# owensgroup/sparsify.me

Measured on AMD Instinct MI355X. Metric: effective GF/s (2:4 spmma vs dense gemm) on ResNet-50 layer shapes, higher is better.
Workload: dtype f16

## Files before the change

### sparsify.me_amd/csrc/mma_tile.h

```cpp
#pragma once
#include "sm_common.h"
#include "select24.h"

namespace sm {

typedef __attribute__((address_space(3))) char lds_char;
typedef __attribute__((address_space(3))) s4 lds_s4;

__device__ __forceinline__ unsigned a_off(unsigned row, unsigned chunk) {
  return row * 128u + 16u * (chunk ^ (row & 7u));
}

__device__ __forceinline__ unsigned b_swz(unsigned kr) { return (((kr >> 1) & 1u) << 1) | (((kr >> 3) & 1u) << 2); }
template <int KROWS>
__device__ __forceinline__ unsigned b_off(unsigned kr, unsigned col ) {
  const unsigned panel = col >> 6, cl = col & 63u;
  return panel * (KROWS * 128u) + kr * 128u + 16u * ((cl >> 3) ^ b_swz(kr)) + 2u * (cl & 7u);
}

template <int KROWS>
__device__ __forceinline__ s4 b_read_tr(const char* Bs, unsigned kr0, unsigned col0, unsigned lane) {
  const unsigned i = lane & 15u, q = i >> 2, p = i & 3u;
  const char* addr = Bs + b_off<KROWS>(kr0 + q, col0 + 4u * p);
  return __builtin_amdgcn_ds_read_tr16_b64_v4i16((lds_s4*)(lds_char*)addr);
// ... 15 lines not shown
}
template <bool BF>
__device__ __forceinline__ f4 smfmac16(h8 a, h16 b, f4 c, int idx) {
  if constexpr (BF) return __builtin_amdgcn_smfmac_f32_16x16x64_bf16(__builtin_bit_cast(bf8, a), __builtin_bit_cast(bf16x16, b), c, idx, 0, 0);
  else return __builtin_amdgcn_smfmac_f32_16x16x64_f16(a, b, c, idx, 0, 0);
}
template <bool BF>
__device__ __forceinline__ f4 mfma16(h8 a, h8 b, f4 c) {
  if constexpr (BF) return __builtin_amdgcn_mfma_f32_16x16x32_bf16(__builtin_bit_cast(bf8, a), __builtin_bit_cast(bf8, b), c, 0, 0, 0);
  else return __builtin_amdgcn_mfma_f32_16x16x32_f16(a, b, c, 0, 0, 0);
}

template <int FM, int FN, bool BF = false>
__device__ __forceinline__ void smfmac_stage(const char* As, const char* Ms, const char* Bs, unsigned row0, unsigned col0,
                                             unsigned lane, f4 (&acc)[FM][FN]) {
  const unsigned g = lane >> 4, r = lane & 15u;
  h8 af[FM];
  int idx[FM];
#pragma unroll
  for (int i = 0; i < FM; ++i) {
    const unsigned row = row0 + i * 16 + r;
    af[i] = *reinterpret_cast<const h8*>(As + row * 64u + 16u * (g ^ a64_swz(row)));
    idx[i] = (int)*reinterpret_cast<const unsigned short*>(Ms + row * 8u + 2u * g);
  }
  const unsigned bs_addr = (unsigned)(uintptr_t)(lds_char*)Bs;
  s4 t0[2], t1[2], t2[2], t3[2];
  auto issue = [&](int j, s4& v0, s4& v1, s4& v2, s4& v3) {
    const unsigned c0 = col0 + j * 16, q = r >> 2, pp = r & 3u;
    const unsigned a = bs_addr + b_off<64>(8u * g + q, c0 + 4u * pp);
    asm volatile("ds_read_b64_tr_b16 %0, %4\n\tds_read_b64_tr_b16 %1, %4 offset:512\n\t"
                 "ds_read_b64_tr_b16 %2, %4 offset:4096\n\tds_read_b64_tr_b16 %3, %4 offset:4608"
                 : "=&v"(v0), "=&v"(v1), "=&v"(v2), "=&v"(v3) : "v"(a) : "memory");
  };
  issue(0, t0[0], t1[0], t2[0], t3[0]);
#pragma unroll
  for (int j = 0; j < FN; ++j) {
    const int c = j & 1, n = c ^ 1;
    if (j + 1 < FN) {
      issue(j + 1, t0[n], t1[n], t2[n], t3[n]);
      asm volatile("s_waitcnt lgkmcnt(4)" : "+v"(t0[c]), "+v"(t1[c]), "+v"(t2[c]), "+v"(t3[c]) :: "memory");
    } else {
      asm volatile("s_waitcnt lgkmcnt(0)" : "+v"(t0[c]), "+v"(t1[c]), "+v"(t2[c]), "+v"(t3[c]) :: "memory");
    }
    __builtin_amdgcn_sched_barrier(0);
    typedef short s16 __attribute__((ext_vector_type(16)));
    const s16 all = {t0[c][0], t0[c][1], t0[c][2], t0[c][3], t1[c][0], t1[c][1], t1[c][2], t1[c][3],
                     t2[c][0], t2[c][1], t2[c][2], t2[c][3], t3[c][0], t3[c][1], t3[c][2], t3[c][3]};
    const h16 bf = __builtin_bit_cast(h16, all);
#pragma unroll
    for (int i = 0; i < FM; ++i) acc[i][j] = smfmac16<BF>(af[i], bf, acc[i][j], idx[i]);
  }
}

template <int FM, int FN, bool BF = false, int D = 1>
__device__ __forceinline__ void smfmac_b_sweep(const h8 (&af)[FM], const int (&idx)[FM], const char* Bs, unsigned col0, unsigned lane,
                                               f4 (&acc)[FM][FN]) {
  static_assert(D == 1 || D == 2, "fragments in flight");
  const unsigned g = lane >> 4, r = lane & 15u;
  const unsigned bs_addr = (unsigned)(uintptr_t)(lds_char*)Bs;
  s4 t0[D + 1], t1[D + 1], t2[D + 1], t3[D + 1];
  auto issue = [&](int j, s4& v0, s4& v1, s4& v2, s4& v3) {
    const unsigned c0 = col0 + j * 16, q = r >> 2, pp = r & 3u;
    const unsigned a = bs_addr + b_off<64>(8u * g + q, c0 + 4u * pp);
    asm volatile("ds_read_b64_tr_b16 %0, %4\n\tds_read_b64_tr_b16 %1, %4 offset:512\n\t"
                 "ds_read_b64_tr_b16 %2, %4 offset:4096\n\tds_read_b64_tr_b16 %3, %4 offset:4608"
                 : "=&v"(v0), "=&v"(v1), "=&v"(v2), "=&v"(v3) : "v"(a) : "memory");
  };
#pragma unroll
  for (int j = 0; j < D; ++j)
    if (j < FN) issue(j, t0[j], t1[j], t2[j], t3[j]);
#pragma unroll
  for (int j = 0; j < FN; ++j) {
    const int c = j % (D + 1), n = (j + D) % (D + 1);
    if (j + D < FN) {
      issue(j + D, t0[n], t1[n], t2[n], t3[n]);
      asm volatile("s_waitcnt lgkmcnt(%4)" : "+v"(t0[c]), "+v"(t1[c]), "+v"(t2[c]), "+v"(t3[c]) : "n"(4 * D) : "memory");
    } else if (D == 2 && j + 1 < FN) {
      asm volatile("s_waitcnt lgkmcnt(4)" : "+v"(t0[c]), "+v"(t1[c]), "+v"(t2[c]), "+v"(t3[c]) :: "memory");
    } else {
      asm volatile("s_waitcnt lgkmcnt(0)" : "+v"(t0[c]), "+v"(t1[c]), "+v"(t2[c]), "+v"(t3[c]) :: "memory");
    }
    __builtin_amdgcn_sched_barrier(0);
    typedef short s16 __attribute__((ext_vector_type(16)));
    const s16 all = {t0[c][0], t0[c][1], t0[c][2], t0[c][3], t1[c][0], t1[c][1], t1[c][2], t1[c][3],
                     t2[c][0], t2[c][1], t2[c][2], t2[c][3], t3[c][0], t3[c][1], t3[c][2], t3[c][3]};
    const h16 bf = __builtin_bit_cast(h16, all);
#pragma unroll
    for (int i = 0; i < FM; ++i) acc[i][j] = smfmac16<BF>(af[i], bf, acc[i][j], idx[i]);
  }
}

__device__ __forceinline__ void dense16_to_operand(const u4 lo, const u4 hi, h8& af, int& idx) {
  uint32_t k0, k1, k2, k3, n0, n1, n2, n3;
  strip_select_f16(lo[0], lo[1], k0, n0);
  strip_select_f16(lo[2], lo[3], k1, n1);
  strip_select_f16(hi[0], hi[1], k2, n2);
  strip_select_f16(hi[2], hi[3], k3, n3);
  af = __builtin_bit_cast(h8, u4{k0, k1, k2, k3});
  idx = (int)(n0 | (n1 << 4) | (n2 << 8) | (n3 << 12));
}

template <int FM, int FN, bool BF = false, int D = 1>
__device__ __forceinline__ void smfmac_stage_dense_a(const char* Araw, const char* Bs, unsigned row0, unsigned col0,
                                                     unsigned lane, f4 (&acc)[FM][FN]) {
  const unsigned g = lane >> 4, r = lane & 15u;
  h8 af[FM];
  int idx[FM];
#pragma unroll
  for (int i = 0; i < FM; ++i) {
    const unsigned row = row0 + i * 16 + r;
    const u4 lo = *reinterpret_cast<const u4*>(Araw + a_off(row, 2u * g));
    const u4 hi = *reinterpret_cast<const u4*>(Araw + a_off(row, 2u * g + 1u));
    dense16_to_operand(lo, hi, af[i], idx[i]);
  }
  smfmac_b_sweep<FM, FN, BF, D>(af, idx, Bs, col0, lane, acc);
}

template <int FM, int FN, bool BF = false>
__device__ __forceinline__ void mfma_b_sweep(const h8 (&a0)[FM], const h8 (&a1)[FM], const char* Bs, unsigned col0, unsigned lane, f4 (&acc)[FM][FN]) {
  const unsigned g = lane >> 4, r = lane & 15u;
  const unsigned bs_addr = (unsigned)(uintptr_t)(lds_char*)Bs;
  s4 t0[2], t1[2], t2[2], t3[2];
  auto issue = [&](int j, s4& v0, s4& v1, s4& v2, s4& v3) {
    const unsigned c0 = col0 + j * 16, q = r >> 2, pp = r & 3u;
    const unsigned a = bs_addr + b_off<64>(8u * g + q, c0 + 4u * pp);
    asm volatile("ds_read_b64_tr_b16 %0, %4\n\tds_read_b64_tr_b16 %1, %4 offset:512\n\t"
                 "ds_read_b64_tr_b16 %2, %4 offset:4096\n\tds_read_b64_tr_b16 %3, %4 offset:4608"
                 : "=&v"(v0), "=&v"(v1), "=&v"(v2), "=&v"(v3) : "v"(a) : "memory");
  };
  issue(0, t0[0], t1[0], t2[0], t3[0]);
#pragma unroll
  for (int j = 0; j < FN; ++j) {
    const int c = j & 1, n = c ^ 1;
    if (j + 1 < FN) {
      issue(j + 1, t0[n], t1[n], t2[n], t3[n]);
      asm volatile("s_waitcnt lgkmcnt(4)" : "+v"(t0[c]), "+v"(t1[c]), "+v"(t2[c]), "+v"(t3[c]) :: "memory");
    } else {
      asm volatile("s_waitcnt lgkmcnt(0)" : "+v"(t0[c]), "+v"(t1[c]), "+v"(t2[c]), "+v"(t3[c]) :: "memory");
    }
    __builtin_amdgcn_sched_barrier(0);
    typedef short s8v __attribute__((ext_vector_type(8)));
    const s8v lo = {t0[c][0], t0[c][1], t0[c][2], t0[c][3], t1[c][0], t1[c][1], t1[c][2], t1[c][3]};
    const s8v hi = {t2[c][0], t2[c][1], t2[c][2], t2[c][3], t3[c][0], t3[c][1], t3[c][2], t3[c][3]};
    const h8 b0 = __builtin_bit_cast(h8, lo), b1 = __builtin_bit_cast(h8, hi);
#pragma unroll
    for (int i = 0; i < FM; ++i) acc[i][j] = mfma16<BF>(a0[i], b0, acc[i][j]);
#pragma unroll
    for (int i = 0; i < FM; ++i) acc[i][j] = mfma16<BF>(a1[i], b1, acc[i][j]);
  }
}
template <int FM, int FN, bool BF = false>
__device__ __forceinline__ void mfma_stage_dense_a(const char* Araw, const char* Bs, unsigned row0, unsigned col0, unsigned lane, f4 (&acc)[FM][FN]) {
  const unsigned g = lane >> 4, r = lane & 15u;
  h8 a0[FM], a1[FM];
#pragma unroll
  for (int i = 0; i < FM; ++i) {
    const unsigned row = row0 + i * 16 + r;
    a0[i] = *reinterpret_cast<const h8*>(Araw + a_off(row, g));
    a1[i] = *reinterpret_cast<const h8*>(Araw + a_off(row, 4u + g));
  }
  mfma_b_sweep<FM, FN, BF>(a0, a1, Bs, col0, lane, acc);
}

template <int BM, int BN, int FM, int FN, int NT, bool BF = false>
__device__ __forceinline__ void store_c_tile(char* smem, half_t* C, const f4 (&acc)[FM][FN], bool has_acc, unsigned row0,
                                             unsigned col0, int m0, int n0, int Mrows, int N, float alpha, float beta,
                                             unsigned tid) {
  constexpr int CPITCH = BN * 2 + 16;
// ... 67 lines not shown
      break;
    case SM_ACT_HARDSWISH:
#pragma unroll
      for (int q = 0; q < 4; ++q) {
        float t = x[q] + 3.0f;
        t = t > 0.0f ? (t < 6.0f ? t : 6.0f) : (t == t ? 0.0f : t);
        y[q] = (x[q] * t) * (1.0f / 6.0f);
      }
      break;
    default: break;
  }
  return y;
}

__device__ __forceinline__ f4 epi_bias4(f4 v, bool bias_col, float bj, bool bias_row, f4 bi) {
#pragma clang fp contract(off)
  if (bias_col) v += bj;
  if (bias_row) v += bi;
  return v;
}

template <int FM, int FN>
struct EpiBias {
  static constexpr int NV = FN > 4 * FM ? FN : 4 * FM;
  float v[NV];
};
template <int FM, int FN>
__device__ __forceinline__ EpiBias<FM, FN> epi_bias_prefetch(const EpiArgs& e, bool has_acc, unsigned row0, unsigned col0, int m0, int n0, int Mrows,
                                                            int N, unsigned lane) {
  EpiBias<FM, FN> eb;
  const unsigned g = lane >> 4, r = lane & 15u;
#pragma unroll
  for (int t = 0; t < EpiBias<FM, FN>::NV; ++t) eb.v[t] = 0.0f;
  if (has_acc && e.bias != nullptr) {
    if (e.bias_dim == SM_BIAS_COL) {
#pragma unroll
      for (int j = 0; j < FN; ++j) {
        const int gc = n0 + (int)(col0 + j * 16 + r);
        if (gc < N) eb.v[j] = e.bias[gc];
      }
    } else {
#pragma unroll
      for (int i = 0; i < FM; ++i)
#pragma unroll
        for (int q = 0; q < 4; ++q) {
          const int gr = m0 + (int)(row0 + i * 16 + 4u * g) + q;
          if (gr < Mrows) eb.v[4 * i + q] = e.bias[gr % e.m];
        }
    }
  }
  return eb;
}

template <int BM, int BN, int FM, int FN, int NT, bool BF = false>
__device__ __forceinline__ void store_c_tile_epi(char* smem, half_t* C, const half_t* R, const EpiArgs& e, const EpiBias<FM, FN>& eb,
                                                 const f4 (&acc)[FM][FN], bool has_acc, unsigned row0, unsigned col0, int m0, int n0,
                                                 int Mrows, int N, float alpha, float beta, unsigned tid) {
  constexpr int CPITCH = BN * 2 + 16;
  const unsigned lane = tid & 63u, g = lane >> 4, r = lane & 15u;
  const bool use_r = beta != 0.0f;
  const bool c_vec = (reinterpret_cast<uintptr_t>(C) & 15u) == 0 && (N % 8 == 0) && (!use_r || (reinterpret_cast<uintptr_t>(R) & 15u) == 0);
  const bool bias_col = e.bias != nullptr && e.bias_dim == SM_BIAS_COL, bias_row = e.bias != nullptr && e.bias_dim == SM_BIAS_ROW;
  constexpr int NCH = BM * (BN / 8);
  if (c_vec) {
    if (use_r) {
      for (unsigned q = tid; q < (unsigned)NCH; q += (unsigned)NT) {
        const unsigned row = q / (BN / 8), cn = q % (BN / 8);
        const int gr = m0 + (int)row, gc = n0 + 8 * (int)cn;
        if (gr >= Mrows || gc >= N) continue;
        *reinterpret_cast<u4*>(smem + row * CPITCH + cn * 16) = __builtin_nontemporal_load(reinterpret_cast<const u4*>(R + (size_t)gr * N + gc));
      }
      __syncthreads();
    }
    if (has_acc) {
#pragma unroll
      for (int i = 0; i < FM; ++i)
#pragma unroll
        for (int j = 0; j < FN; ++j) {
          const unsigned row = row0 + i * 16 + 4u * g, col = col0 + j * 16 + r;
          f4 v4;
#pragma unroll
          for (int q = 0; q < 4; ++q) {
            float v = alpha * acc[i][j][q];
            if (use_r) v += beta * to_f32<BF>(*reinterpret_cast<const half_t*>(smem + (row + q) * CPITCH + col * 2));
            v4[q] = v;
          }
          v4 = epi_act4(epi_bias4(v4, bias_col, eb.v[j < EpiBias<FM, FN>::NV ? j : 0], bias_row, f4{eb.v[4 * i], eb.v[4 * i + 1], eb.v[4 * i + 2], eb.v[4 * i + 3]}), e.act, e.act_arg);
#pragma unroll
          for (int q = 0; q < 4; ++q) *reinterpret_cast<half_t*>(smem + (row + q) * CPITCH + col * 2) = to_elt<BF>(v4[q]);
        }
    }
    __syncthreads();
    for (unsigned q = tid; q < (unsigned)NCH; q += (unsigned)NT) {
      const unsigned row = q / (BN / 8), cn = q % (BN / 8);
      const int gr = m0 + (int)row, gc = n0 + 8 * (int)cn;
      if (gr >= Mrows || gc >= N) continue;
      __builtin_nontemporal_store(*reinterpret_cast<const u4*>(smem + row * CPITCH + cn * 16), reinterpret_cast<u4*>(C + (size_t)gr * N + gc));
    }
  } else if (has_acc) {
#pragma unroll
    for (int i = 0; i < FM; ++i)
#pragma unroll
      for (int j = 0; j < FN; ++j) {
        const int gc = n0 + (int)(col0 + j * 16 + r);
        if (gc >= N) continue;
        f4 v4;
#pragma unroll
        for (int q = 0; q < 4; ++q) {
          const int gr = m0 + (int)(row0 + i * 16 + 4u * g) + q;
          float v = alpha * acc[i][j][q];
          if (use_r && gr < Mrows) v += beta * to_f32<BF>(R[(size_t)gr * N + gc]);
          v4[q] = v;
        }
        v4 = epi_act4(epi_bias4(v4, bias_col, eb.v[j < EpiBias<FM, FN>::NV ? j : 0], bias_row, f4{eb.v[4 * i], eb.v[4 * i + 1], eb.v[4 * i + 2], eb.v[4 * i + 3]}), e.act, e.act_arg);
#pragma unroll
        for (int q = 0; q < 4; ++q) {
          const int gr = m0 + (int)(row0 + i * 16 + 4u * g) + q;
          if (gr < Mrows) C[(size_t)gr * N + gc] = to_elt<BF>(v4[q]);
        }
      }
  }
}

__device__ __forceinline__ unsigned xcd_remap(unsigned id, unsigned nwg) {
  const unsigned q = nwg >> 3, r = nwg & 7u, x = id & 7u;
  const unsigned base = x < r ? x * (q + 1u) : r * (q + 1u) + (x - r) * q;
  return base + (id >> 3);
}

__device__ __forceinline__ unsigned tile_order(unsigned id, unsigned nwg, bool dispatch_order) { return dispatch_order ? id : xcd_remap(id, nwg); }

typedef __attribute__((address_space(1))) const void gptr_t;
typedef __attribute__((address_space(3))) void lptr_t;

template <int N>
__device__ __forceinline__ void wait_dma_and_barrier() {
  asm volatile("s_waitcnt vmcnt(%0)\n\ts_barrier" ::"n"(N) : "memory");
}

}
```

### sparsify.me_amd/csrc/spmma_f16_fused.hip

```cpp
#include "select24.h"
#include "spmma_args.h"

namespace sm {

constexpr int MAXG = 8;
struct FusedArgs {
  const half_t* A[MAXG];
  const half_t* B[MAXG];
  half_t* C[MAXG];
  size_t sA, sB, sC;
  int Mrows, N, K, lda;
  int batch, tiles_m, tiles_n;
  int ngroup;
  float alpha, beta;
  const half_t* const* dAp;
  const half_t* const* dBp;
  half_t* const* dCp;
};

struct FusedArgsEpi : FusedArgs {
  EpiArgs e;
};
template <bool EPI> struct FusedArgsSel { typedef FusedArgs type; };
template <> struct FusedArgsSel<true> { typedef FusedArgsEpi type; };
// ... 61 lines not shown
  };

  f4 acc[FM][FN];
#pragma unroll
  for (int i = 0; i < FM; ++i)
#pragma unroll
    for (int j = 0; j < FN; ++j) acc[i][j] = f4{0.f, 0.f, 0.f, 0.f};

#pragma unroll
  for (int s = 0; s < NS - 1; ++s)
    if (s < nkt) stage(s, s);
  int cur = 0, fill = NS - 1;
  for (int kt = 0; kt < nkt; ++kt) {
    const int ahead = (nkt - 1 - kt) < (NS - 2) ? (nkt - 1 - kt) : (NS - 2);
    if (NS >= 4 && ahead == 2) wait_dma_and_barrier<2 * SL>();
    else if (NS >= 3 && ahead == 1) wait_dma_and_barrier<SL>();
    else wait_dma_and_barrier<0>();
    if (kt + NS - 1 < nkt) stage(kt + NS - 1, fill);
    const char* As = smem + cur * STAGE;
    if constexpr (DENSE) mfma_stage_dense_a<FM, FN, BF>(As, As + SA, wave * TM, 0, lane, acc);
    else smfmac_stage_dense_a<FM, FN, BF>(As, As + SA, wave * TM, 0, lane, acc);
    cur = cur + 1 == NS ? 0 : cur + 1;
    fill = fill + 1 == NS ? 0 : fill + 1;
  }
  __syncthreads();
  if constexpr (EPI) store_c_tile_epi<BM, BN, FM, FN, 64 * NW, BF>(smem, C, p.e.R + (size_t)b * p.e.sR, p.e, eb, acc, true, wave * TM, 0, m0, n0, p.Mrows, p.N, p.alpha, p.beta, tid);
  else store_c_tile<BM, BN, FM, FN, 64 * NW, BF>(smem, C, acc, true, wave * TM, 0, m0, n0, p.Mrows, p.N, p.alpha, p.beta, tid);
}

template <int BN, int NS, bool BF = false, int BM = 128, int NWV = 4, bool ANT = true, bool DENSE = false, bool EPI = false>
static int launch_fused_direct(const typename FusedArgsSel<EPI>::type& a0, hipStream_t st) {
  typename FusedArgsSel<EPI>::type a = a0;
  a.tiles_m = (a.Mrows + BM - 1) / BM;
  a.tiles_n = (a.N + BN - 1) / BN;
  const size_t nwg = (size_t)a.tiles_m * a.tiles_n * a.batch * a.ngroup;
  if (nwg == 0) return SM_STATUS_SUCCESS;
  if (nwg > 0x7fffffffu) {
    set_error("sm_spmma_fused_f16: grid too large");
    return SM_STATUS_NOT_SUPPORTED;
  }
  constexpr size_t stage_bytes = BM * 128 + 64 * BN * 2;
  const size_t lds_main = ((size_t)(a.K / 64) < (size_t)NS ? (size_t)(a.K / 64) : (size_t)NS) * stage_bytes;
  constexpr size_t lds_epi = (size_t)BM * (BN * 2 + 16);
  const size_t lds = lds_main > lds_epi ? lds_main : lds_epi;
  constexpr size_t lds_max = NS * stage_bytes > lds_epi ? NS * stage_bytes : lds_epi;
  static LdsOptIn lds_optin;
  if (lds_max > 64 * 1024) {
    if (const int rc = ensure_dyn_lds(lds_optin, reinterpret_cast<const void*>(&spmma_f16_fused_direct_kernel<BN, NS, BF, BM, NWV, ANT, DENSE, EPI>), lds_max, "spmma_f16_fused_direct_kernel")) return rc;
  }
  spmma_f16_fused_direct_kernel<BN, NS, BF, BM, NWV, ANT, DENSE, EPI><<<dim3((unsigned)nwg), dim3(64 * NWV), lds, st>>>(a);
  return check_launch("spmma_f16_fused_direct_kernel");
}

template <int BN, bool BF = false, int NSA = 3, int NSB = 2, bool ANT = true, bool DENSE = false, bool EPI = false>
__global__ __launch_bounds__(512) void spmma_f16_fused_big_kernel(const typename FusedArgsSel<EPI>::type p) {
  constexpr int BM = 256, NW = 8, TM = BM / NW, FM = TM / 16, FN = BN / 16;
  constexpr int SA = BM * 128, SB = 64 * BN * 2;
  constexpr int A_N = BM / 8, B_N = BN / 8;
  static_assert(A_N % NW == 0 && B_N % NW == 0, "equal DMA share per wave");
  static_assert(NSA == 3 && (NSB == 2 || NSB == 3), "ring depths the counted waits below are written for");
  constexpr int SLA = A_N / NW, SLB = B_N / NW;
  constexpr int AHEAD = SLA + (NSB == 3 ? SLB : 0);
  constexpr int BRING = NSA * SA;
  extern __shared__ __attribute__((aligned(16))) char smem[];

  const unsigned tid = threadIdx.x, lane = tid & 63u;
  const unsigned wave = __builtin_amdgcn_readfirstlane(tid >> 6);
  const unsigned tiles = (unsigned)p.tiles_m * (unsigned)p.tiles_n;
  const unsigned lid = xcd_remap(blockIdx.x, gridDim.x);
  const unsigned gb = lid / tiles, trem = lid - gb * tiles;
  const unsigned grp = gb / (unsigned)p.batch, b = gb - grp * (unsigned)p.batch;
  const unsigned tile_m = trem / (unsigned)p.tiles_n, tile_n = trem - tile_m * (unsigned)p.tiles_n;
  const int m0 = (int)tile_m * BM, n0 = (int)tile_n * BN;
  const int nkt = p.K / 64;
  const half_t* A = p.dAp ? p.dAp[gb] : p.A[grp] + (size_t)b * p.sA;
  const half_t* B = p.dBp ? p.dBp[gb] : p.B[grp] + (size_t)b * p.sB;
  half_t* C = p.dCp ? p.dCp[gb] : p.C[grp] + (size_t)b * p.sC;
  const int mlast = p.Mrows - 1;
  EpiBias<FM, FN> eb;
  if constexpr (EPI) eb = epi_bias_prefetch<FM, FN>(p.e, true, wave * TM, 0, m0, n0, p.Mrows, p.N, lane);

  const char* asrc[SLA];
  const char* bsrc[SLB];
  unsigned aoff[SLA], boff[SLB];
#pragma unroll
  for (int i = 0; i < SLA; ++i) {
    const unsigned t = wave + (unsigned)NW * i;
    const unsigned row = 8u * t + (lane >> 3), cs = (lane & 7u) ^ (row & 7u);
    int gr = m0 + (int)row;
    gr = gr < mlast ? gr : mlast;
    asrc[i] = reinterpret_cast<const char*>(A + (size_t)gr * p.lda) + 16u * cs;
    aoff[i] = t * 1024u;
  }
#pragma unroll
  for (int i = 0; i < SLB; ++i) {
    const unsigned j = wave + (unsigned)NW * i, panel = j >> 3, kr = 8u * (j & 7u) + (lane >> 3);
    const unsigned cs = (lane & 7u) ^ b_swz(kr);
    int gc = n0 + (int)(64u * panel + 8u * cs);
    gc = gc <= p.N - 8 ? gc : p.N - 8;
    bsrc[i] = reinterpret_cast<const char*>(B + (size_t)kr * p.N + gc);
    boff[i] = BRING + panel * 8192u + (j & 7u) * 1024u;
  }
  const size_t bstep = (size_t)64 * p.N * 2;
  auto stage_a = [&](int kt, int buf) {
#pragma unroll
    for (int i = 0; i < SLA; ++i) {
      if (ANT) __builtin_amdgcn_global_load_lds((gptr_t*)(asrc[i] + (size_t)kt * 128), (lptr_t*)(smem + buf * SA + aoff[i]), 16, 0, 2);
      else __builtin_amdgcn_global_load_lds((gptr_t*)(asrc[i] + (size_t)kt * 128), (lptr_t*)(smem + buf * SA + aoff[i]), 16, 0, 0);
    }
  };
  auto stage_b = [&](int kt, int buf) {
#pragma unroll
    for (int i = 0; i < SLB; ++i)
      __builtin_amdgcn_global_load_lds((gptr_t*)(bsrc[i] + (size_t)kt * bstep), (lptr_t*)(smem + buf * SB + boff[i]), 16, 0, 0);
  };

  f4 acc[FM][FN];
#pragma unroll
  for (int i = 0; i < FM; ++i)
#pragma unroll
    for (int j = 0; j < FN; ++j) acc[i][j] = f4{0.f, 0.f, 0.f, 0.f};

#pragma unroll
  for (int j = -(NSA - 1); j < 0; ++j) {
    if (j + NSB - 1 >= 0 && j + NSB - 1 < nkt) stage_b(j + NSB - 1, j + NSB - 1);
    if (j + NSA - 1 < nkt) stage_a(j + NSA - 1, j + NSA - 1);
  }
  int ca = 0, cb = 0, fa = NSA - 1, fb = NSB - 1;
  for (int kt = 0; kt < nkt; ++kt) {
    if (kt + 1 < nkt) wait_dma_and_barrier<AHEAD>();
    else wait_dma_and_barrier<0>();
    if (kt + NSB - 1 < nkt) stage_b(kt + NSB - 1, fb);
    if (kt + NSA - 1 < nkt) stage_a(kt + NSA - 1, fa);
    if constexpr (DENSE) mfma_stage_dense_a<FM, FN, BF>(smem + ca * SA, smem + BRING + cb * SB, wave * TM, 0, lane, acc);
    else smfmac_stage_dense_a<FM, FN, BF>(smem + ca * SA, smem + BRING + cb * SB, wave * TM, 0, lane, acc);
    ca = ca + 1 == NSA ? 0 : ca + 1;
    fa = fa + 1 == NSA ? 0 : fa + 1;
    cb = cb + 1 == NSB ? 0 : cb + 1;
    fb = fb + 1 == NSB ? 0 : fb + 1;
  }
  __syncthreads();
  if constexpr (EPI) store_c_tile_epi<BM, BN, FM, FN, 64 * NW, BF>(smem, C, p.e.R + (size_t)b * p.e.sR, p.e, eb, acc, true, wave * TM, 0, m0, n0, p.Mrows, p.N, p.alpha, p.beta, tid);
  else store_c_tile<BM, BN, FM, FN, 64 * NW, BF>(smem, C, acc, true, wave * TM, 0, m0, n0, p.Mrows, p.N, p.alpha, p.beta, tid);
}

template <int BN, bool BF = false, int NSA = 3, int NSB = 2, bool ANT = true, bool DENSE = false, bool EPI = false>
static int launch_fused_big(const typename FusedArgsSel<EPI>::type& a0, hipStream_t st) {
  constexpr int BM = 256;
  typename FusedArgsSel<EPI>::type a = a0;
  a.tiles_m = (a.Mrows + BM - 1) / BM;
  a.tiles_n = (a.N + BN - 1) / BN;
  const size_t nwg = (size_t)a.tiles_m * a.tiles_n * a.batch * a.ngroup;
  if (nwg == 0) return SM_STATUS_SUCCESS;
  if (nwg > 0x7fffffffu) {
    set_error("sm_spmma_fused_f16: grid too large");
    return SM_STATUS_NOT_SUPPORTED;
  }
  constexpr size_t lds_main = (size_t)NSA * BM * 128 + (size_t)NSB * 64 * BN * 2;
  constexpr size_t lds_epi = (size_t)BM * (BN * 2 + 16);
  constexpr size_t lds = lds_main > lds_epi ? lds_main : lds_epi;
  static_assert(lds <= 160 * 1024, "LDS budget of the big direct kernel");
  static LdsOptIn lds_optin;
  if (const int rc = ensure_dyn_lds(lds_optin, reinterpret_cast<const void*>(&spmma_f16_fused_big_kernel<BN, BF, NSA, NSB, ANT, DENSE, EPI>), lds, "spmma_f16_fused_big_kernel")) return rc;
  spmma_f16_fused_big_kernel<BN, BF, NSA, NSB, ANT, DENSE, EPI><<<dim3((unsigned)nwg), dim3(512), lds, st>>>(a);
  return check_launch("spmma_f16_fused_big_kernel");
}

template <class T>
__device__ __forceinline__ T* sk_uniform(T* ptr) {
  const unsigned long long v = reinterpret_cast<unsigned long long>(ptr);
  const unsigned lo = __builtin_amdgcn_readfirstlane((unsigned)v), hi = __builtin_amdgcn_readfirstlane((unsigned)(v >> 32));
  return reinterpret_cast<T*>(((unsigned long long)hi << 32) | lo);
}


struct SkArgs {
  float* part;
  unsigned* flags;
  unsigned panels, slots, tg, wg, groups_full, tgl, wgl;
  unsigned cut[9], cutl[9];
};
__device__ __forceinline__ unsigned sk_pick(const unsigned (&tab)[9], unsigned r) {
  unsigned v = tab[0];
#pragma unroll
  for (unsigned i = 1; i < 9; ++i) v = r == i ? tab[i] : v;
  return v;
}
__device__ __forceinline__ unsigned long long sk_slot_start(const SkArgs& s, unsigned w, unsigned nkt) {
  const unsigned q = w / s.wg;
  if (q < s.groups_full) return ((unsigned long long)q * s.tg) * nkt + sk_pick(s.cut, w - q * s.wg);
  unsigned r = w - s.groups_full * s.wg;
  r = r < s.wgl ? r : s.wgl;
  return ((unsigned long long)s.groups_full * s.tg) * nkt + (s.wgl ? sk_pick(s.cutl, r) : 0u);
}
__device__ __forceinline__ void sk_store_sc1(float* dst, f4 v) {
  asm volatile("global_store_dwordx4 %0, %1, off sc1" ::"v"(dst), "v"(v) : "memory");
}
__device__ __forceinline__ f4 sk_load_sc1(const float* src) {
  f4 v;
  asm volatile("global_load_dwordx4 %0, %1, off sc1" : "=v"(v) : "v"(src) : "memory");
  return v;
}

template <int BN, bool BF = false, bool ANT = true, bool DENSE = false>
__global__ __launch_bounds__(512) void spmma_f16_fused_sk_kernel(const FusedArgs p, const SkArgs s) {
  constexpr int BM = 256, NW = 8, TM = BM / NW, FM = TM / 16, FN = BN / 16, NSA = 3, NSB = 2;
  constexpr int SA = BM * 128, SB = 64 * BN * 2;
  constexpr int A_N = BM / 8, B_N = BN / 8;
  static_assert(A_N % NW == 0 && B_N % NW == 0, "equal DMA share per wave");
  constexpr int SLA = A_N / NW, SLB = B_N / NW;
  constexpr int AHEAD = SLA;
  constexpr int BRING = NSA * SA;
  extern __shared__ __attribute__((aligned(16))) char smem[];

  const unsigned tid = threadIdx.x, lane = tid & 63u;
  const unsigned wave = __builtin_amdgcn_readfirstlane(tid >> 6);
  const unsigned lid = xcd_remap(blockIdx.x, gridDim.x);
  const unsigned tn = (unsigned)p.tiles_n;
  const unsigned slot = lid / tn, tile_n = lid - slot * tn;
  const unsigned nkt = (unsigned)(p.K / 64);
  const unsigned long long u0 = sk_slot_start(s, slot, nkt), u1 = sk_slot_start(s, slot + 1u, nkt);
  const int mlast = p.Mrows - 1;
  const size_t bstep = (size_t)64 * p.N * 2;
  const size_t slot_floats = (size_t)BM * BN;

  bool publish_pending = false;
// ... 1116 lines not shown
}

template <bool BF>
static int spmma_fused16(size_t ngroup, const void* const* Ag, const void* const* Bg, void* const* Cg, size_t m, size_t n, size_t k, size_t lda,
                         size_t batch, size_t strideA, size_t strideB, size_t strideC, float alpha, float beta,
                         sm_stream_t stream, void* workspace = nullptr, size_t workspace_bytes = 0, const EpiArgs* epi = nullptr) {
#define SM_LAUNCH(fn, ...) (epi ? fn<__VA_ARGS__, true>(ae, st) : fn<__VA_ARGS__, false>(a, st))
  if (ngroup == 0) return SM_STATUS_SUCCESS;
  if (!Ag || !Bg || !Cg || lda < k || ngroup > (size_t)MAXG) {
    set_error("sm_spmma_fused_{f16,bf16}: invalid argument");
    return SM_STATUS_INVALID_VALUE;
  }
  FusedCall c = {m, n, k, lda, batch, ngroup, strideA, strideB, strideC, beta, true, true, true, workspace != nullptr, aligned16(workspace), workspace_bytes,
                 epi != nullptr, epi && aligned16(epi->R), epi ? epi->sR : 0};
  for (size_t g = 0; g < ngroup; ++g) {
    if (!Ag[g] || !Bg[g] || !Cg[g]) {
      set_error("sm_spmma_fused_{f16,bf16}: invalid argument (null operand)");
      return SM_STATUS_INVALID_VALUE;
    }
    c.a_aligned = c.a_aligned && aligned16(Ag[g]);
    c.b_aligned = c.b_aligned && aligned16(Bg[g]);
    c.c_aligned = c.c_aligned && aligned16(Cg[g]);
  }
  const FusedPick pick = fused_form(c, (size_t)device_cu_count());
  hipStream_t st = (hipStream_t)stream;
  FusedArgs a = {};
  for (size_t g = 0; g < (size_t)MAXG; ++g) {
    const size_t s_ = g < ngroup ? g : 0;
    a.A[g] = (const half_t*)Ag[s_]; a.B[g] = (const half_t*)Bg[s_]; a.C[g] = (half_t*)Cg[s_];
  }
  a.ngroup = (int)ngroup;
  a.N = (int)n; a.K = (int)k; a.lda = (int)lda;
  a.alpha = alpha; a.beta = beta;
  if (pick.stacked) {
    a.Mrows = (int)(m * batch);
    a.batch = 1;
  } else {
    a.Mrows = (int)m;
    a.batch = (int)batch;
  }
  if (pick.form != SM_FUSED_FORM_SPAN) { a.sA = strideA; a.sB = strideB; a.sC = strideC; }
  FusedArgsEpi ae = {};
  static_cast<FusedArgs&>(ae) = a;
  if (epi) ae.e = *epi;
  switch (pick.form) {
    case SM_FUSED_FORM_EMPTY: return SM_STATUS_SUCCESS;
    case SM_FUSED_FORM_NOT_TAKEN:
      set_error("%s", pick.why);
      return SM_STATUS_NOT_SUPPORTED;
    case SM_FUSED_FORM_THIN: return spmma_fused_thin(BF, (int)ngroup, Ag, Bg, Cg, m * batch, n, k, alpha, beta, st);
    case SM_FUSED_FORM_SPAN: return n <= 64 ? SM_LAUNCH(launch_fused_span, 64, BF, false) : SM_LAUNCH(launch_fused_span, 128, BF, false);
    case SM_FUSED_FORM_STREAMK:
      return n <= 256 ? launch_fused_sk<256, BF, true>(a, workspace, workspace_bytes, st) : launch_fused_sk<256, BF, false>(a, workspace, workspace_bytes, st);
    case SM_FUSED_FORM_BIG: return n <= 256 ? SM_LAUNCH(launch_fused_big, 256, BF, 3, 2, true, false) : SM_LAUNCH(launch_fused_big, 256, BF, 3, 2, false, false);
    case SM_FUSED_FORM_DIRECT64: return SM_LAUNCH(launch_fused_direct, 64, 2, BF, 128, 4, true, false);
    case SM_FUSED_FORM_DIRECT128: return SM_LAUNCH(launch_fused_direct, 128, 2, BF, 128, 4, false, false);
    case SM_FUSED_FORM_DIRECT128_NT: return SM_LAUNCH(launch_fused_direct, 128, 2, BF, 128, 4, true, false);
    case SM_FUSED_FORM_ASTAT: return launch_fused_astat<BF>(a, st);
    case SM_FUSED_FORM_WIDEP: return launch_fused_widep<256, 4, 2, 4, 2, 3, BF>(a, st);
    case SM_FUSED_FORM_WIDE: return SM_LAUNCH(launch_fused_wide, 256, 4, 2, 4, 2, 3, BF, false);
    case SM_FUSED_FORM_WIDE_NT: return SM_LAUNCH(launch_fused_wide, 256, 4, 2, 4, 2, 3, BF, true);
  }
  set_error("sm_spmma_fused_{f16,bf16}: internal error (unknown form)");
  return SM_STATUS_LAUNCH_FAILED;
#undef SM_LAUNCH
}

extern "C" int sm_spmma_fused_f16(const void* A, const void* B, void* C, size_t m, size_t n, size_t k, size_t lda,
                                  size_t batch, size_t strideA, size_t strideB, size_t strideC, float alpha, float beta,
                                  sm_stream_t stream) {
  return spmma_fused16<false>(1, &A, &B, &C, m, n, k, lda, batch, strideA, strideB, strideC, alpha, beta, stream);
}
extern "C" int sm_spmma_fused_bf16(const void* A, const void* B, void* C, size_t m, size_t n, size_t k, size_t lda,
                                   size_t batch, size_t strideA, size_t strideB, size_t strideC, float alpha, float beta,
                                   sm_stream_t stream) {
  return spmma_fused16<true>(1, &A, &B, &C, m, n, k, lda, batch, strideA, strideB, strideC, alpha, beta, stream);
}

template <bool BF>
static int spmma_fused16_ex(const void* A, const void* B, void* D, size_t m, size_t n, size_t k, size_t lda, size_t batch, size_t strideA, size_t strideB,
                            size_t strideD, float alpha, float beta, const sm_epilogue_t* ep, sm_stream_t stream) {
  EpiArgs e;
  bool plain;
  if (const int rc = epilogue_args(ep, D, strideD, m, beta, e, &plain, "sm_spmma_fused_{f16,bf16}_ex")) return rc;
  return spmma_fused16<BF>(1, &A, &B, &D, m, n, k, lda, batch, strideA, strideB, strideD, alpha, beta, stream, nullptr, 0, plain ? nullptr : &e);
}
extern "C" int sm_spmma_fused_f16_ex(const void* A, const void* B, void* D, size_t m, size_t n, size_t k, size_t lda, size_t batch,
                                     size_t strideA, size_t strideB, size_t strideD, float alpha, float beta, const sm_epilogue_t* epilogue,
                                     sm_stream_t stream) {
  return spmma_fused16_ex<false>(A, B, D, m, n, k, lda, batch, strideA, strideB, strideD, alpha, beta, epilogue, stream);
}
extern "C" int sm_spmma_fused_bf16_ex(const void* A, const void* B, void* D, size_t m, size_t n, size_t k, size_t lda, size_t batch,
                                      size_t strideA, size_t strideB, size_t strideD, float alpha, float beta, const sm_epilogue_t* epilogue,
                                      sm_stream_t stream) {
  return spmma_fused16_ex<true>(A, B, D, m, n, k, lda, batch, strideA, strideB, strideD, alpha, beta, epilogue, stream);
}

extern "C" int sm_spmma_fused_workspace_size(size_t* bytes) {
  if (!bytes) {
    set_error("sm_spmma_fused_workspace_size: invalid argument");
    return SM_STATUS_INVALID_VALUE;
  }
  *bytes = sk_workspace_bytes((size_t)device_cu_count(), 256);
  return SM_STATUS_SUCCESS;
}
extern "C" int sm_spmma_fused_workspace_state(const void* workspace, int* state, sm_stream_t stream) {
  if (!workspace || !state) {
// ... 106 lines not shown
```

Before: 573,900.

## Add dedicated DMA loader waves to big fused spmma kernel (warp specialization)

The big fused kernel gains four extra loader waves (NDW=4) that issue all global-to-LDS DMA and drive the ring waits. The eight compute waves now only run barriers and smfmac sweeps, and the B-operand address math is simplified with an XOR-based offset. Bias values are handed from a loader wave to the epilogue through LDS. The aim is to take DMA issue and address arithmetic off the compute waves so the MFMA work overlaps better, at the cost of more threads per workgroup, lower occupancy and extra barrier coupling.

```diff
diff --git a/sparsify.me_amd/csrc/mma_tile.h b/sparsify.me_amd/csrc/mma_tile.h
--- a/sparsify.me_amd/csrc/mma_tile.h
+++ b/sparsify.me_amd/csrc/mma_tile.h
@@ -91,7 +91,7 @@
   }
 }
 
-template <int FM, int FN, bool BF = false, int D = 1>
+template <int FM, int FN, bool BF = false, int D = 1, bool XA = false>
 __device__ __forceinline__ void smfmac_b_sweep(const h8 (&af)[FM], const int (&idx)[FM], const char* Bs, unsigned col0, unsigned lane,
                                                f4 (&acc)[FM][FN]) {
   static_assert(D == 1 || D == 2, "fragments in flight");
@@ -100,7 +100,12 @@
   s4 t0[D + 1], t1[D + 1], t2[D + 1], t3[D + 1];
   auto issue = [&](int j, s4& v0, s4& v1, s4& v2, s4& v3) {
     const unsigned c0 = col0 + j * 16, q = r >> 2, pp = r & 3u;
-    const unsigned a = bs_addr + b_off<64>(8u * g + q, c0 + 4u * pp);
+    unsigned a = bs_addr + b_off<64>(8u * g + q, c0 + 4u * pp);
+    if constexpr (XA) {
+      unsigned off0 = b_off<64>(8u * g + q, col0 + 4u * pp);
+      asm volatile("" : "+v"(off0));
+      a = bs_addr + (unsigned)(j >> 2) * 8192u + (off0 ^ (32u * (unsigned)(j & 3)));
+    }
     asm volatile("ds_read_b64_tr_b16 %0, %4\n\tds_read_b64_tr_b16 %1, %4 offset:512\n\t"
                  "ds_read_b64_tr_b16 %2, %4 offset:4096\n\tds_read_b64_tr_b16 %3, %4 offset:4608"
                  : "=&v"(v0), "=&v"(v1), "=&v"(v2), "=&v"(v3) : "v"(a) : "memory");
@@ -139,7 +144,7 @@
   idx = (int)(n0 | (n1 << 4) | (n2 << 8) | (n3 << 12));
 }
 
-template <int FM, int FN, bool BF = false, int D = 1>
+template <int FM, int FN, bool BF = false, int D = 1, bool XA = false>
 __device__ __forceinline__ void smfmac_stage_dense_a(const char* Araw, const char* Bs, unsigned row0, unsigned col0,
                                                      unsigned lane, f4 (&acc)[FM][FN]) {
   const unsigned g = lane >> 4, r = lane & 15u;
@@ -152,7 +157,7 @@
     const u4 hi = *reinterpret_cast<const u4*>(Araw + a_off(row, 2u * g + 1u));
     dense16_to_operand(lo, hi, af[i], idx[i]);
   }
-  smfmac_b_sweep<FM, FN, BF, D>(af, idx, Bs, col0, lane, acc);
+  smfmac_b_sweep<FM, FN, BF, D, XA>(af, idx, Bs, col0, lane, acc);
 }
 
 template <int FM, int FN, bool BF = false>
@@ -326,16 +331,32 @@
   return eb;
 }
 
-template <int BM, int BN, int FM, int FN, int NT, bool BF = false>
+template <int BM, int BN, int FM, int FN, int NT, bool BF = false, bool BL = false>
 __device__ __forceinline__ void store_c_tile_epi(char* smem, half_t* C, const half_t* R, const EpiArgs& e, const EpiBias<FM, FN>& eb,
                                                  const f4 (&acc)[FM][FN], bool has_acc, unsigned row0, unsigned col0, int m0, int n0,
-                                                 int Mrows, int N, float alpha, float beta, unsigned tid) {
+                                                 int Mrows, int N, float alpha, float beta, unsigned tid, const float* bl = nullptr) {
   constexpr int CPITCH = BN * 2 + 16;
   const unsigned lane = tid & 63u, g = lane >> 4, r = lane & 15u;
   const bool use_r = beta != 0.0f;
   const bool c_vec = (reinterpret_cast<uintptr_t>(C) & 15u) == 0 && (N % 8 == 0) && (!use_r || (reinterpret_cast<uintptr_t>(R) & 15u) == 0);
   const bool bias_col = e.bias != nullptr && e.bias_dim == SM_BIAS_COL, bias_row = e.bias != nullptr && e.bias_dim == SM_BIAS_ROW;
   constexpr int NCH = BM * (BN / 8);
+  auto bias_j = [&](int j) -> float {
+    if constexpr (BL) {
+      unsigned r_ = r;
+      asm volatile("" : "+v"(r_));
+      return bias_col ? bl[col0 + j * 16 + r_] : 0.0f;
+    }
+    else return eb.v[j < EpiBias<FM, FN>::NV ? j : 0];
+  };
+  auto bias_i = [&](int i) -> f4 {
+    if constexpr (BL) {
+      unsigned g_ = g;
+      asm volatile("" : "+v"(g_));
+      return bias_row ? *reinterpret_cast<const f4*>(bl + row0 + i * 16 + 4u * g_) : f4{0.f, 0.f, 0.f, 0.f};
+    }
+    else return f4{eb.v[4 * i], eb.v[4 * i + 1], eb.v[4 * i + 2], eb.v[4 * i + 3]};
+  };
   if (c_vec) {
     if (use_r) {
       for (unsigned q = tid; q < (unsigned)NCH; q += (unsigned)NT) {
@@ -359,9 +380,10 @@
             if (use_r) v += beta * to_f32<BF>(*reinterpret_cast<const half_t*>(smem + (row + q) * CPITCH + col * 2));
             v4[q] = v;
           }
-          v4 = epi_act4(epi_bias4(v4, bias_col, eb.v[j < EpiBias<FM, FN>::NV ? j : 0], bias_row, f4{eb.v[4 * i], eb.v[4 * i + 1], eb.v[4 * i + 2], eb.v[4 * i + 3]}), e.act, e.act_arg);
+          v4 = epi_act4(epi_bias4(v4, bias_col, bias_j(j), bias_row, bias_i(i)), e.act, e.act_arg);
 #pragma unroll
           for (int q = 0; q < 4; ++q) *reinterpret_cast<half_t*>(smem + (row + q) * CPITCH + col * 2) = to_elt<BF>(v4[q]);
+          if constexpr (BL) __builtin_amdgcn_sched_barrier(0);
         }
     }
     __syncthreads();
@@ -378,20 +400,23 @@
       for (int j = 0; j < FN; ++j) {
         const int gc = n0 + (int)(col0 + j * 16 + r);
         if (gc >= N) continue;
+        unsigned g4 = 4u * g;
+        if constexpr (BL) asm volatile("" : "+v"(g4));
         f4 v4;
 #pragma unroll
         for (int q = 0; q < 4; ++q) {
-          const int gr = m0 + (int)(row0 + i * 16 + 4u * g) + q;
+          const int gr = m0 + (int)(row0 + i * 16 + g4) + q;
           float v = alpha * acc[i][j][q];
           if (use_r && gr < Mrows) v += beta * to_f32<BF>(R[(size_t)gr * N + gc]);
           v4[q] = v;
         }
-        v4 = epi_act4(epi_bias4(v4, bias_col, eb.v[j < EpiBias<FM, FN>::NV ? j : 0], bias_row, f4{eb.v[4 * i], eb.v[4 * i + 1], eb.v[4 * i + 2], eb.v[4 * i + 3]}), e.act, e.act_arg);
+        v4 = epi_act4(epi_bias4(v4, bias_col, bias_j(j), bias_row, bias_i(i)), e.act, e.act_arg);
 #pragma unroll
         for (int q = 0; q < 4; ++q) {
-          const int gr = m0 + (int)(row0 + i * 16 + 4u * g) + q;
+          const int gr = m0 + (int)(row0 + i * 16 + g4) + q;
           if (gr < Mrows) C[(size_t)gr * N + gc] = to_elt<BF>(v4[q]);
         }
+        if constexpr (BL) __builtin_amdgcn_sched_barrier(0);
       }
   }
 }
diff --git a/sparsify.me_amd/csrc/spmma_f16_fused.hip b/sparsify.me_amd/csrc/spmma_f16_fused.hip
--- a/sparsify.me_amd/csrc/spmma_f16_fused.hip
+++ b/sparsify.me_amd/csrc/spmma_f16_fused.hip
@@ -137,15 +137,67 @@
   return check_launch("spmma_f16_fused_direct_kernel");
 }
 
-template <int BN, bool BF = false, int NSA = 3, int NSB = 2, bool ANT = true, bool DENSE = false, bool EPI = false>
-__global__ __launch_bounds__(512) void spmma_f16_fused_big_kernel(const typename FusedArgsSel<EPI>::type p) {
+template <class T>
+__device__ __forceinline__ T* sk_uniform(T* ptr) {
+  const unsigned long long v = reinterpret_cast<unsigned long long>(ptr);
+  const unsigned lo = __builtin_amdgcn_readfirstlane((unsigned)v), hi = __builtin_amdgcn_readfirstlane((unsigned)(v >> 32));
+  return reinterpret_cast<T*>(((unsigned long long)hi << 32) | lo);
+}
+template <int BN, int NL, int NSA, bool ANT>
+struct BigDma {
+  static constexpr int BM = 256, SA = BM * 128, SB = 64 * BN * 2, BRING = NSA * SA;
+  static constexpr int SLA = BM / 8 / NL, SLB = BN / 8 / NL;
+  const char* asrc[SLA];
+  const char* bsrc[SLB];
+  unsigned aoff[SLA], boff[SLB];
+  size_t bstep;
+  __device__ __forceinline__ void init(const half_t* A, const half_t* B, unsigned lw, unsigned lane, int m0, int n0, int mlast, int N, int lda) {
+#pragma unroll
+    for (int i = 0; i < SLA; ++i) {
+      const unsigned t = lw + (unsigned)NL * i;
+      const unsigned row = 8u * t + (lane >> 3), cs = (lane & 7u) ^ (row & 7u);
+      int gr = m0 + (int)row;
+      gr = gr < mlast ? gr : mlast;
+      asrc[i] = reinterpret_cast<const char*>(A + (size_t)gr * lda) + 16u * cs;
+      aoff[i] = t * 1024u;
+    }
+#pragma unroll
+    for (int i = 0; i < SLB; ++i) {
+      const unsigned j = lw + (unsigned)NL * i, panel = j >> 3, kr = 8u * (j & 7u) + (lane >> 3);
+      const unsigned cs = (lane & 7u) ^ b_swz(kr);
+      int gc = n0 + (int)(64u * panel + 8u * cs);
+      gc = gc <= N - 8 ? gc : N - 8;
+      bsrc[i] = reinterpret_cast<const char*>(B + (size_t)kr * N + gc);
+      boff[i] = BRING + panel * 8192u + (j & 7u) * 1024u;
+    }
+    bstep = (size_t)64 * N * 2;
+  }
+  __device__ __forceinline__ void stage_a(char* smem, int kt, int buf) const {
+#pragma unroll
+    for (int i = 0; i < SLA; ++i) {
+      if (ANT) __builtin_amdgcn_global_load_lds((gptr_t*)(asrc[i] + (size_t)kt * 128), (lptr_t*)(smem + buf * SA + aoff[i]), 16, 0, 2);
+      else __builtin_amdgcn_global_load_lds((gptr_t*)(asrc[i] + (size_t)kt * 128), (lptr_t*)(smem + buf * SA + aoff[i]), 16, 0, 0);
+    }
+  }
+  __device__ __forceinline__ void stage_b(char* smem, int kt, int buf) const {
+#pragma unroll
+    for (int i = 0; i < SLB; ++i)
+      __builtin_amdgcn_global_load_lds((gptr_t*)(bsrc[i] + (size_t)kt * bstep), (lptr_t*)(smem + buf * SB + boff[i]), 16, 0, 0);
+  }
+};
+
+template <int BN, bool BF = false, int NSA = 3, int NSB = 2, bool ANT = true, bool DENSE = false, int NDW = 0, bool EPI = false>
+__global__ __launch_bounds__(64 * (8 + NDW)) void spmma_f16_fused_big_kernel(const typename FusedArgsSel<EPI>::type p) {
   constexpr int BM = 256, NW = 8, TM = BM / NW, FM = TM / 16, FN = BN / 16;
   constexpr int SA = BM * 128, SB = 64 * BN * 2;
   constexpr int A_N = BM / 8, B_N = BN / 8;
-  static_assert(A_N % NW == 0 && B_N % NW == 0, "equal DMA share per wave");
+  constexpr int NL = NDW ? NDW : NW;
+  static_assert(NDW == 0 || NDW == 4, "loader waves");
+  static_assert(A_N % NL == 0 && B_N % NL == 0, "equal DMA share per wave");
   static_assert(NSA == 3 && (NSB == 2 || NSB == 3), "ring depths the counted waits below are written for");
-  constexpr int SLA = A_N / NW, SLB = B_N / NW;
+  constexpr int SLA = A_N / NL, SLB = B_N / NL;
   constexpr int AHEAD = SLA + (NSB == 3 ? SLB : 0);
+  static_assert(AHEAD < 64, "vmcnt field");
   constexpr int BRING = NSA * SA;
   extern __shared__ __attribute__((aligned(16))) char smem[];
 
@@ -162,74 +214,88 @@
   const half_t* B = p.dBp ? p.dBp[gb] : p.B[grp] + (size_t)b * p.sB;
   half_t* C = p.dCp ? p.dCp[gb] : p.C[grp] + (size_t)b * p.sC;
   const int mlast = p.Mrows - 1;
-  EpiBias<FM, FN> eb;
-  if constexpr (EPI) eb = epi_bias_prefetch<FM, FN>(p.e, true, wave * TM, 0, m0, n0, p.Mrows, p.N, lane);
-
-  const char* asrc[SLA];
-  const char* bsrc[SLB];
-  unsigned aoff[SLA], boff[SLB];
-#pragma unroll
-  for (int i = 0; i < SLA; ++i) {
-    const unsigned t = wave + (unsigned)NW * i;
-    const unsigned row = 8u * t + (lane >> 3), cs = (lane & 7u) ^ (row & 7u);
-    int gr = m0 + (int)row;
-    gr = gr < mlast ? gr : mlast;
-    asrc[i] = reinterpret_cast<const char*>(A + (size_t)gr * p.lda) + 16u * cs;
-    aoff[i] = t * 1024u;
-  }
-#pragma unroll
-  for (int i = 0; i < SLB; ++i) {
-    const unsigned j = wave + (unsigned)NW * i, panel = j >> 3, kr = 8u * (j & 7u) + (lane >> 3);
-    const unsigned cs = (lane & 7u) ^ b_swz(kr);
-    int gc = n0 + (int)(64u * panel + 8u * cs);
-    gc = gc <= p.N - 8 ? gc : p.N - 8;
-    bsrc[i] = reinterpret_cast<const char*>(B + (size_t)kr * p.N + gc);
-    boff[i] = BRING + panel * 8192u + (j & 7u) * 1024u;
-  }
-  const size_t bstep = (size_t)64 * p.N * 2;
-  auto stage_a = [&](int kt, int buf) {
-#pragma unroll
-    for (int i = 0; i < SLA; ++i) {
-      if (ANT) __builtin_amdgcn_global_load_lds((gptr_t*)(asrc[i] + (size_t)kt * 128), (lptr_t*)(smem + buf * SA + aoff[i]), 16, 0, 2);
-      else __builtin_amdgcn_global_load_lds((gptr_t*)(asrc[i] + (size_t)kt * 128), (lptr_t*)(smem + buf * SA + aoff[i]), 16, 0, 0);
-    }
+  const bool has_acc = NDW == 0 || wave < (unsigned)NW;
+  if constexpr (NDW != 0) C = sk_uniform(C);
+  const unsigned bu = NDW == 0 ? b : __builtin_amdgcn_readfirstlane(b);
+  EpiBias<FM, FN> eb = {};
+  constexpr int BIAS_OFF = BM * (BN * 2 + 16);
+  static_assert(NDW == 0 || !EPI || BIAS_OFF + BM * 4 <= NSA * SA + NSB * SB, "the bias hand-off lies inside the rings' LDS");
+  static_assert(BM == BN, "one bias value per lane element either way");
+  f4 lbias;
+  if constexpr (EPI && NDW == 0) eb = epi_bias_prefetch<FM, FN>(p.e, has_acc, wave * TM, 0, m0, n0, p.Mrows, p.N, lane);
+
+  f4 acc[FM][FN];
+  auto zero_acc = [&]() {
+#pragma unroll
+    for (int i = 0; i < FM; ++i)
+#pragma unroll
+      for (int j = 0; j < FN; ++j) acc[i][j] = f4{0.f, 0.f, 0.f, 0.f};
   };
-  auto stage_b = [&](int kt, int buf) {
-#pragma unroll
-    for (int i = 0; i < SLB; ++i)
-      __builtin_amdgcn_global_load_lds((gptr_t*)(bsrc[i] + (size_t)kt * bstep), (lptr_t*)(smem + buf * SB + boff[i]), 16, 0, 0);
+  auto compute = [&](int ca, int cb) {
+    if constexpr (DENSE) mfma_stage_dense_a<FM, FN, BF>(smem + ca * SA, smem + BRING + cb * SB, wave * TM, 0, lane, acc);
+    else smfmac_stage_dense_a<FM, FN, BF, 1, NDW != 0>(smem + ca * SA, smem + BRING + cb * SB, wave * TM, 0, lane, acc);
   };
 
-  f4 acc[FM][FN];
-#pragma unroll
-  for (int i = 0; i < FM; ++i)
-#pragma unroll
-    for (int j = 0; j < FN; ++j) acc[i][j] = f4{0.f, 0.f, 0.f, 0.f};
-
-#pragma unroll
-  for (int j = -(NSA - 1); j < 0; ++j) {
-    if (j + NSB - 1 >= 0 && j + NSB - 1 < nkt) stage_b(j + NSB - 1, j + NSB - 1);
-    if (j + NSA - 1 < nkt) stage_a(j + NSA - 1, j + NSA - 1);
-  }
-  int ca = 0, cb = 0, fa = NSA - 1, fb = NSB - 1;
-  for (int kt = 0; kt < nkt; ++kt) {
-    if (kt + 1 < nkt) wait_dma_and_barrier<AHEAD>();
-    else wait_dma_and_barrier<0>();
-    if (kt + NSB - 1 < nkt) stage_b(kt + NSB - 1, fb);
-    if (kt + NSA - 1 < nkt) stage_a(kt + NSA - 1, fa);
-    if constexpr (DENSE) mfma_stage_dense_a<FM, FN, BF>(smem + ca * SA, smem + BRING + cb * SB, wave * TM, 0, lane, acc);
-    else smfmac_stage_dense_a<FM, FN, BF>(smem + ca * SA, smem + BRING + cb * SB, wave * TM, 0, lane, acc);
-    ca = ca + 1 == NSA ? 0 : ca + 1;
-    fa = fa + 1 == NSA ? 0 : fa + 1;
-    cb = cb + 1 == NSB ? 0 : cb + 1;
-    fb = fb + 1 == NSB ? 0 : fb + 1;
+  if (NDW == 0 || !has_acc) {
+    BigDma<BN, NL, NSA, ANT> d;
+    d.init(A, B, NDW ? wave - (unsigned)NW : wave, lane, m0, n0, mlast, p.N, p.lda);
+    if constexpr (NDW == 0) zero_acc();
+    if constexpr (EPI && NDW != 0) {
+      lbias = f4{0.f, 0.f, 0.f, 0.f};
+      if (wave == (unsigned)NW && p.e.bias != nullptr) {
+#pragma unroll
+        for (int q = 0; q < 4; ++q) {
+          const int x = 4 * (int)lane + q;
+          if (p.e.bias_dim == SM_BIAS_COL) {
+            if (n0 + x < p.N) lbias[q] = p.e.bias[n0 + x];
+          } else if (m0 + x < p.Mrows) lbias[q] = p.e.bias[(m0 + x) % p.e.m];
+        }
+      }
+    }
+#pragma unroll
+    for (int j = -(NSA - 1); j < 0; ++j) {
+      if (j + NSB - 1 >= 0 && j + NSB - 1 < nkt) d.stage_b(smem, j + NSB - 1, j + NSB - 1);
+      if (j + NSA - 1 < nkt) d.stage_a(smem, j + NSA - 1, j + NSA - 1);
+    }
+    int ca = 0, cb = 0, fa = NSA - 1, fb = NSB - 1;
+    for (int kt = 0; kt < nkt; ++kt) {
+      if (kt + 1 < nkt) wait_dma_and_barrier<AHEAD>();
+      else wait_dma_and_barrier<0>();
+      if (kt + NSB - 1 < nkt) d.stage_b(smem, kt + NSB - 1, fb);
+      if (kt + NSA - 1 < nkt) d.stage_a(smem, kt + NSA - 1, fa);
+      if constexpr (NDW == 0) compute(ca, cb);
+      ca = ca + 1 == NSA ? 0 : ca + 1;
+      fa = fa + 1 == NSA ? 0 : fa + 1;
+      cb = cb + 1 == NSB ? 0 : cb + 1;
+      fb = fb + 1 == NSB ? 0 : fb + 1;
+    }
+    if constexpr (NDW != 0) zero_acc();
+  } else {
+    zero_acc();
+    int ca = 0, cb = 0;
+    for (int kt = 0; kt < nkt; ++kt) {
+      asm volatile("s_barrier" ::: "memory");
+      compute(ca, cb);
+      ca = ca + 1 == NSA ? 0 : ca + 1;
+      cb = cb + 1 == NSB ? 0 : cb + 1;
+    }
+    if constexpr (EPI && NDW != 0) lbias = f4{0.f, 0.f, 0.f, 0.f};
   }
   __syncthreads();
-  if constexpr (EPI) store_c_tile_epi<BM, BN, FM, FN, 64 * NW, BF>(smem, C, p.e.R + (size_t)b * p.e.sR, p.e, eb, acc, true, wave * TM, 0, m0, n0, p.Mrows, p.N, p.alpha, p.beta, tid);
-  else store_c_tile<BM, BN, FM, FN, 64 * NW, BF>(smem, C, acc, true, wave * TM, 0, m0, n0, p.Mrows, p.N, p.alpha, p.beta, tid);
-}
-
-template <int BN, bool BF = false, int NSA = 3, int NSB = 2, bool ANT = true, bool DENSE = false, bool EPI = false>
+  constexpr int NT = 64 * (NW + NDW);
+  const unsigned tid_e = NDW == 0 ? tid : wave * 64u + __builtin_amdgcn_mbcnt_hi(~0u, __builtin_amdgcn_mbcnt_lo(~0u, 0u));
+  if constexpr (EPI && NDW != 0) {
+    float* bl = reinterpret_cast<float*>(smem + BIAS_OFF);
+    const unsigned le = tid_e & 63u;
+    if (wave == (unsigned)NW) *reinterpret_cast<f4*>(bl + 4u * le) = lbias;
+    __syncthreads();
+    store_c_tile_epi<BM, BN, FM, FN, NT, BF, true>(smem, C, p.e.R + (size_t)bu * p.e.sR, p.e, eb, acc, has_acc, wave * TM, 0, m0, n0, p.Mrows, p.N, p.alpha, p.beta, tid_e, bl);
+  } else
+  if constexpr (EPI) store_c_tile_epi<BM, BN, FM, FN, NT, BF>(smem, C, p.e.R + (size_t)b * p.e.sR, p.e, eb, acc, has_acc, wave * TM, 0, m0, n0, p.Mrows, p.N, p.alpha, p.beta, tid_e);
+  else store_c_tile<BM, BN, FM, FN, NT, BF>(smem, C, acc, has_acc, wave * TM, 0, m0, n0, p.Mrows, p.N, p.alpha, p.beta, tid_e);
+}
+
+template <int BN, bool BF = false, int NSA = 3, int NSB = 2, bool ANT = true, bool DENSE = false, int NDW = 0, bool EPI = false>
 static int launch_fused_big(const typename FusedArgsSel<EPI>::type& a0, hipStream_t st) {
   constexpr int BM = 256;
   typename FusedArgsSel<EPI>::type a = a0;
@@ -246,17 +312,11 @@
   constexpr size_t lds = lds_main > lds_epi ? lds_main : lds_epi;
   static_assert(lds <= 160 * 1024, "LDS budget of the big direct kernel");
   static LdsOptIn lds_optin;
-  if (const int rc = ensure_dyn_lds(lds_optin, reinterpret_cast<const void*>(&spmma_f16_fused_big_kernel<BN, BF, NSA, NSB, ANT, DENSE, EPI>), lds, "spmma_f16_fused_big_kernel")) return rc;
-  spmma_f16_fused_big_kernel<BN, BF, NSA, NSB, ANT, DENSE, EPI><<<dim3((unsigned)nwg), dim3(512), lds, st>>>(a);
+  if (const int rc = ensure_dyn_lds(lds_optin, reinterpret_cast<const void*>(&spmma_f16_fused_big_kernel<BN, BF, NSA, NSB, ANT, DENSE, NDW, EPI>), lds, "spmma_f16_fused_big_kernel")) return rc;
+  spmma_f16_fused_big_kernel<BN, BF, NSA, NSB, ANT, DENSE, NDW, EPI><<<dim3((unsigned)nwg), dim3(64 * (8 + NDW)), lds, st>>>(a);
   return check_launch("spmma_f16_fused_big_kernel");
 }
 
-template <class T>
-__device__ __forceinline__ T* sk_uniform(T* ptr) {
-  const unsigned long long v = reinterpret_cast<unsigned long long>(ptr);
-  const unsigned lo = __builtin_amdgcn_readfirstlane((unsigned)v), hi = __builtin_amdgcn_readfirstlane((unsigned)(v >> 32));
-  return reinterpret_cast<T*>(((unsigned long long)hi << 32) | lo);
-}
 
 
 struct SkArgs {
@@ -1479,7 +1539,7 @@
     case SM_FUSED_FORM_SPAN: return n <= 64 ? SM_LAUNCH(launch_fused_span, 64, BF, false) : SM_LAUNCH(launch_fused_span, 128, BF, false);
     case SM_FUSED_FORM_STREAMK:
       return n <= 256 ? launch_fused_sk<256, BF, true>(a, workspace, workspace_bytes, st) : launch_fused_sk<256, BF, false>(a, workspace, workspace_bytes, st);
-    case SM_FUSED_FORM_BIG: return n <= 256 ? SM_LAUNCH(launch_fused_big, 256, BF, 3, 2, true, false) : SM_LAUNCH(launch_fused_big, 256, BF, 3, 2, false, false);
+    case SM_FUSED_FORM_BIG: return n <= 256 ? SM_LAUNCH(launch_fused_big, 256, BF, 3, 2, true, false, 4) : SM_LAUNCH(launch_fused_big, 256, BF, 3, 2, false, false, 4);
     case SM_FUSED_FORM_DIRECT64: return SM_LAUNCH(launch_fused_direct, 64, 2, BF, 128, 4, true, false);
     case SM_FUSED_FORM_DIRECT128: return SM_LAUNCH(launch_fused_direct, 128, 2, BF, 128, 4, false, false);
     case SM_FUSED_FORM_DIRECT128_NT: return SM_LAUNCH(launch_fused_direct, 128, 2, BF, 128, 4, true, false);
```

Result: no change. 578,500, median of 6 (+0.8%).
